# SuperScientificSoftwareLaboratory/TileSpMV

Measured on AMD Instinct MI355X. Metric: fp64 SpMV GFLOP/s (y = A*x, tiled format), higher is better.
Workload: dtype f64; 1 GPU; laplacian4096; rows=16777216, cols=16777216, nnz=83869696, partition=tile-row blocks, nnz-balanced, 1 rank(s), y_combine=none, tiles=5234176, x_panel_merge=0, x_slice_passes=0

## Files before the change

include/tilespmv.h:

```cpp
#ifndef TILESPMV_H_
#define TILESPMV_H_

#include <stddef.h>
#include <stdint.h>

#ifdef __cplusplus
extern "C" {
#endif

#ifndef MAT_VAL_TYPE
#define MAT_VAL_TYPE double
#endif
#ifndef MAT_PTR_TYPE
#define MAT_PTR_TYPE int
#endif

#define TILESPMV_BLOCK_SIZE 16
#define TILESPMV_COO_NNZ_TH 12
#define TILESPMV_PREFETCH_SMEM_TH 4

enum {
    TILESPMV_FMT_CSR = 0,
    TILESPMV_FMT_COO = 1,
    TILESPMV_FMT_ELL = 2,
// ... 240 lines not shown
    TILESPMV_INFO_WG_STRIPS = 16,
    TILESPMV_INFO_LIST_ENTRIES = 17,
    TILESPMV_INFO_DERIVED_UNITS = 18,
    TILESPMV_INFO_BRICK_ORDER = 19,
    TILESPMV_INFO_DESC_BYTES = 20,
    TILESPMV_INFO_NT_STREAM = 21,
    TILESPMV_INFO_UNIT_VALUE_BYTES = 22,
    TILESPMV_INFO_UNIT_LEAN = 23,
    TILESPMV_INFO_PLACEMENT_TRIES = 24,
    TILESPMV_INFO_RETIRED_25 = 25,
    TILESPMV_INFO_X_PANELS = 26,
    TILESPMV_INFO_X_PANEL_MERGE = 27,
    TILESPMV_INFO_SCATTERED_ENTRIES = 28,
    TILESPMV_INFO_X_SLICE_PASSES = 29,
    TILESPMV_INFO_CSR_FORM = 30,
    TILESPMV_INFO_TIMED_CHOICES_US = 31,
    TILESPMV_INFO_DEVICE_BUILD = 32,
    TILESPMV_INFO_TILE_CREATE_US = 33,
    TILESPMV_INFO_VALUE_MAP_BYTES = 34,
    TILESPMV_INFO_COUNT = 35
};
void tilespmv_plan_info(const tilespmv_plan *plan, long long *out );
int tilespmv_plan_strip_stride(const tilespmv_plan *plan);
long long tilespmv_plan_stream_digests(const tilespmv_plan *plan, unsigned long long *out , long long max_streams);

double tilespmv_plan_time(tilespmv_plan *plan, const MAT_VAL_TYPE *d_x, MAT_VAL_TYPE *d_y,
                          void *stream, int warmup, int reps);

double tilespmv_plan_time_reference_style(tilespmv_plan *plan, const MAT_VAL_TYPE *d_x, MAT_VAL_TYPE *d_y,
                                          void *stream, int reps);

void tilespmv_partition_tilerows(const Tile_matrix *matrix, int nparts, int *bounds);

int tilespmv_sizeof_value(void);

int tilespmv_reorder_rcm(int n, const MAT_PTR_TYPE *csrRowPtr, const int *csrColIdx, int *perm );
int tilespmv_csr_permute(int n, const MAT_PTR_TYPE *csrRowPtr, const int *csrColIdx, const MAT_VAL_TYPE *csrVal, const int *perm,
                         MAT_PTR_TYPE *outRowPtr , int *outColIdx, MAT_VAL_TYPE *outVal);
long long tilespmv_csr_bandwidth(int n, const MAT_PTR_TYPE *csrRowPtr, const int *csrColIdx);
int tilespmv_permute_vector(const MAT_VAL_TYPE *d_in, MAT_VAL_TYPE *d_out, const int *d_perm, long long n, int scatter, void *stream);

int tilespmv_csr_transpose(int rowA, int colA, const MAT_PTR_TYPE *csrRowPtr, const int *csrColIdx, const MAT_VAL_TYPE *csrVal ,
                           MAT_PTR_TYPE *rowPtrT , int *colIdxT, MAT_VAL_TYPE *valT , int *srcT );
int tilespmv_csr_transpose_device(int rowA, int colA, const MAT_PTR_TYPE *d_csrRowPtr, const int *d_csrColIdx, const MAT_VAL_TYPE *d_csrVal ,
                                  MAT_PTR_TYPE *d_rowPtrT, int *d_colIdxT, MAT_VAL_TYPE *d_valT , int *d_srcT , void *stream);

// ... 119 lines not shown
```

tilespmv_amd/_lib.py:

```python
import ctypes as C
import os
import subprocess

import numpy as np

from .tile_matrix import TileMatrixF32, TileMatrixF64

_ROOT = os.path.dirname(os.path.abspath(__file__))
_I = C.POINTER(C.c_int)
_U = C.POINTER(C.c_uint)
_CACHE = {}

INFO_NAMES = ["device_bytes", "stream_bytes", "nnz", "rows", "tiles", "coo_mode", "dense_mode", "kernel",
              "num_tasks", "num_split_rows", "fallback_nnz", "build_us", "upload_us", "entry_mode", "entry_ordered", "strip_cost",
              "wg_strips", "list_entries", "derived_units", "brick_order", "desc_bytes", "nt_stream", "unit_value_bytes", "unit_lean", "placement_tries", "retired_25", "x_panels", "x_panel_merge", "scattered_entries", "x_slice_passes", "csr_form", "timed_choices_us", "device_build", "tile_create_us",
              "value_map_bytes"]


BJ_INFO_NAMES = ["rows", "block_size", "blocks", "singular_blocks", "device_bytes", "dot_partials"]

FSAI_INFO_NAMES = ["rows", "nnz", "longest_row", "truncated_rows", "fallback_rows", "device_bytes", "dot_partials"]

KNOB_DEFAULT = -1
KNOB_NAMES = ["entry_mode", "entry_ordered", "strip_cost", "split_above", "split_cap", "xcd_remap", "xcd_chunk", "csr_split", "fix_inline",
# ... 94 lines not shown
    lib.tilespmv_plan_spmm.argtypes = [C.c_void_p, C.c_void_p, C.c_void_p, C.c_int, C.c_void_p]
    lib.tilespmv_plan_spmm.restype = C.c_int
    lib.tilespmv_plan_time_spmm.argtypes = [C.c_void_p, C.c_void_p, C.c_void_p, C.c_int, C.c_void_p, C.c_int, C.c_int]
    lib.tilespmv_plan_time_spmm.restype = C.c_double
    lib.tilespmv_plan_create.argtypes = [C.POINTER(C.c_void_p), TP, C.c_int, C.c_int, C.c_int, C.POINTER(PlanOptions)]
    lib.tilespmv_plan_create.restype = C.c_int
    lib.tilespmv_plan_options_init.argtypes = [C.POINTER(PlanOptions)]
    lib.tilespmv_plan_options_init.restype = None
    lib.tilespmv_plan_layout_digest.argtypes = [TP, C.c_int, C.c_int, C.c_int, C.POINTER(PlanOptions), C.POINTER(C.c_ulonglong), C.POINTER(C.c_longlong)]
    lib.tilespmv_plan_layout_digest.restype = C.c_int
    lib.tilespmv_plan_layout_stages.argtypes = [TP, C.c_int, C.c_int, C.c_int, C.POINTER(PlanOptions), C.POINTER(C.c_ulonglong), C.POINTER(C.c_longlong)]
    lib.tilespmv_plan_layout_stages.restype = C.c_int
    lib.tilespmv_plan_destroy.argtypes = [C.c_void_p]
    lib.tilespmv_plan_destroy.restype = None
    lib.tilespmv_plan_spmv.argtypes = [C.c_void_p, C.c_void_p, C.c_void_p, C.c_void_p]
    lib.tilespmv_plan_spmv.restype = C.c_int
    lib.tilespmv_plan_spmv_n.argtypes = [C.c_void_p, C.c_void_p, C.c_void_p, C.c_void_p, C.c_int]
    lib.tilespmv_plan_spmv_n.restype = C.c_int
    lib.tilespmv_plan_info.argtypes = [C.c_void_p, C.POINTER(C.c_longlong)]
    lib.tilespmv_plan_info.restype = None
    if hasattr(lib, "tilespmv_plan_strip_stride"):
        lib.tilespmv_plan_strip_stride.argtypes = [C.c_void_p]
        lib.tilespmv_plan_strip_stride.restype = C.c_int
    lib.tilespmv_plan_time.argtypes = [C.c_void_p, C.c_void_p, C.c_void_p, C.c_void_p, C.c_int, C.c_int]
    lib.tilespmv_plan_time.restype = C.c_double
    lib.tilespmv_plan_time_reference_style.argtypes = [C.c_void_p, C.c_void_p, C.c_void_p, C.c_void_p, C.c_int]
    lib.tilespmv_plan_time_reference_style.restype = C.c_double
    lib.tilespmv_plan_reserve_spmm.argtypes = [C.c_void_p, C.c_int]
    lib.tilespmv_plan_reserve_spmm.restype = C.c_int
    lib.tilespmv_partition_tilerows.argtypes = [TP, C.c_int, _I]
    lib.tilespmv_partition_tilerows.restype = None
    lib.tilespmv_matrix_save.argtypes = [TP, C.c_int, C.c_int, C.c_int, C.c_char_p]
    lib.tilespmv_matrix_save.restype = C.c_int
    lib.tilespmv_matrix_load.argtypes = [TP, _I, _I, _I, C.c_char_p]
    lib.tilespmv_matrix_load.restype = C.c_int
    lib.tilespmv_csr_save.argtypes = [C.c_char_p, C.c_int, C.c_int, C.c_int, C.c_int, _I, _I, VP, C.c_char_p]
    lib.tilespmv_csr_save.restype = C.c_int
    lib.tilespmv_csr_load.argtypes = [C.c_char_p, _I, _I, _I, _I, C.POINTER(_I), C.POINTER(_I), C.POINTER(VP), C.c_char_p]
    lib.tilespmv_csr_load.restype = C.c_int
    lib.mmio_allinone_cached.argtypes = [_I, _I, _I, _I, C.POINTER(_I), C.POINTER(_I), C.POINTER(VP), C.c_char_p, C.c_char_p, _I]
    lib.mmio_allinone_cached.restype = C.c_int
    lib.tilespmv_mtx_write.argtypes = [C.c_char_p, C.c_int, C.c_int, C.c_int, _I, _I, VP]
    lib.tilespmv_mtx_write.restype = C.c_int
    lib.tilespmv_reorder_rcm.argtypes = [C.c_int, _I, _I, _I]
    lib.tilespmv_reorder_rcm.restype = C.c_int
    lib.tilespmv_csr_permute.argtypes = [C.c_int, _I, _I, VP, _I, _I, _I, VP]
# ... 83 lines not shown
                    "tilespmv_device_count", "tilespmv_matrix_save", "tilespmv_matrix_load", "tilespmv_plan_spmv_n",
                    "call_tilespmv_hip_multi", "tilespmv_plan_spmm", "tilespmv_plan_time_spmm", "tilespmv_plan_options_init", "tilespmv_plan_layout_digest",
                    "tilespmv_csr_save", "tilespmv_csr_load", "mmio_allinone_cached", "tilespmv_mtx_write",
                    "tilespmv_plan_time_reference_style", "tilespmv_plan_reserve_spmm", "tilespmv_plan_options_layout", "tilespmv_plan_layout_stages",
                    "Tile_create_device", "tilespmv_plan_create_from_csr", "tilespmv_plan_stream_digests", "tilespmv_plan_create_from_device_csr",
                    "tilespmv_reorder_rcm", "tilespmv_csr_permute", "tilespmv_csr_bandwidth", "tilespmv_permute_vector",
                    "tilespmv_plan_update_values", "tilespmv_csr_transpose", "tilespmv_csr_transpose_device",
                    "tilespmv_cg_create", "tilespmv_cg_destroy", "tilespmv_cg_begin", "tilespmv_cg_iterate", "tilespmv_cg_state_read", "tilespmv_cg_solve",
                    "tilespmv_csr_diagonal_device",
                    "tilespmv_cg_multi_create", "tilespmv_cg_multi_destroy", "tilespmv_cg_multi_begin", "tilespmv_cg_multi_iterate", "tilespmv_cg_multi_state_read",
                    "tilespmv_cg_multi_solve",
                    "tilespmv_cgls_create", "tilespmv_cgls_destroy", "tilespmv_cgls_begin", "tilespmv_cgls_iterate", "tilespmv_cgls_state_read", "tilespmv_cgls_solve",
                    "tilespmv_csr_row_sqnorms_device",
                    "tilespmv_bicgstab_create", "tilespmv_bicgstab_destroy", "tilespmv_bicgstab_begin", "tilespmv_bicgstab_iterate", "tilespmv_bicgstab_state_read",
                    "tilespmv_bicgstab_solve",
                    "tilespmv_minres_create", "tilespmv_minres_destroy", "tilespmv_minres_begin", "tilespmv_minres_iterate", "tilespmv_minres_state_read", "tilespmv_minres_solve",
                    "tilespmv_csr_abs_diagonal_device",
                    "tilespmv_block_jacobi_create", "tilespmv_block_jacobi_destroy", "tilespmv_block_jacobi_update", "tilespmv_block_jacobi_apply", "tilespmv_block_jacobi_apply_dot",
                    "tilespmv_block_jacobi_info", "tilespmv_cg_create_block", "tilespmv_bicgstab_create_block",
                    "tilespmv_fsai_create", "tilespmv_fsai_destroy", "tilespmv_fsai_update", "tilespmv_fsai_apply", "tilespmv_fsai_apply_dot", "tilespmv_fsai_factor_csr",
                    "tilespmv_fsai_info", "tilespmv_cg_create_fsai",
                    "tilespmv_gmres_create", "tilespmv_gmres_create_block", "tilespmv_gmres_destroy", "tilespmv_gmres_begin", "tilespmv_gmres_iterate", "tilespmv_gmres_flush",
                    "tilespmv_gmres_state_read", "tilespmv_gmres_solve", "tilespmv_gmres_create_basis", "tilespmv_gmres_basis_bytes", "tilespmv_gmres_workspace_bytes",
                    "tilespmv_plan_strip_stride"]
```

tilespmv_amd/api.py:

```python
import ctypes as C

import numpy as np

from . import _lib
from .tile_matrix import to_dict

_I, _U = _lib._I, _lib._U

COO_AUTO, COO_IN_TILE, COO_FALLBACK = 0, 1, 2
DENSE_AUTO, DENSE_MFMA, DENSE_VALU = 0, 1, 2
KERNEL_AUTO, KERNEL_DIRECT, KERNEL_STREAM = 0, 1, 2
CREATE_HYB, CREATE_QUIET, CREATE_CDNA4, CREATE_VALUE_MAP = 1, 2, 4, 8
CREATE_TRANSPOSE = 16
ERR_NO_VALUE_MAP = -4


def _p(a, t):
    return a.ctypes.data_as(C.POINTER(t))


def _take(lib, ptr, n, dtype):
    if not ptr:
        return np.zeros(0, dtype=dtype)
    addr = C.cast(ptr, C.c_void_p).value
# ... 199 lines not shown

def csr_bandwidth(n, rowptr, colidx, dtype=np.float64):
    lib = _lib.load(dtype)
    rp, ci = np.ascontiguousarray(rowptr, dtype=np.int32), np.ascontiguousarray(colidx, dtype=np.int32)
    return int(lib.tilespmv_csr_bandwidth(n, _p(rp, C.c_int), _p(ci, C.c_int)))


def permute_vector(d_in, d_out, d_perm, n, scatter=False, stream=0, dtype=np.float64):
    rc = _lib.load(dtype).tilespmv_permute_vector(d_in, d_out, d_perm, n, 1 if scatter else 0, stream)
    if rc != 0:
        raise RuntimeError("tilespmv_permute_vector failed (hipError %d)" % rc)


def plan_layout_digest(tm, rowA, colA, nnzA, coo_mode=COO_AUTO, dense_mode=DENSE_AUTO, kernel=0, tilerow_begin=0, tilerow_end=0, **knobs):
    opts = _lib.PlanOptions(coo_mode, dense_mode, kernel, tilerow_begin, tilerow_end, False, **knobs)
    d = C.c_ulonglong(0)
    out = (C.c_longlong * len(_lib.INFO_NAMES))()
    rc = tm._lib.tilespmv_plan_layout_digest(C.byref(tm), rowA, colA, nnzA, C.byref(opts), C.byref(d), out)
    if rc != 0:
        raise RuntimeError("tilespmv_plan_layout_digest failed (%d)" % rc)
    return d.value, {k: int(out[i]) for i, k in enumerate(_lib.INFO_NAMES)}


STAGE_NAMES = ["count", "choose", "cut", "emit", "order", "encode", "entries", "finish"]


def plan_layout_stages(tm, rowA, colA, nnzA, coo_mode=COO_AUTO, dense_mode=DENSE_AUTO, kernel=0, tilerow_begin=0, tilerow_end=0, **knobs):
    opts = _lib.PlanOptions(coo_mode, dense_mode, kernel, tilerow_begin, tilerow_end, False, **knobs)
    st = (C.c_ulonglong * len(STAGE_NAMES))()
    out = (C.c_longlong * len(_lib.INFO_NAMES))()
    rc = tm._lib.tilespmv_plan_layout_stages(C.byref(tm), rowA, colA, nnzA, C.byref(opts), st, out)
    if rc != 0:
        raise RuntimeError("tilespmv_plan_layout_stages failed (%d)" % rc)
    return {k: int(st[i]) for i, k in enumerate(STAGE_NAMES)}, {k: int(out[i]) for i, k in enumerate(_lib.INFO_NAMES)}


class Plan:

    def __init__(self, tm, rowA, colA, nnzA, coo_mode=COO_AUTO, dense_mode=DENSE_AUTO, kernel=0, tilerow_begin=0, tilerow_end=0, autotune=False, **knobs):
        self.lib = tm._lib
        self.rowA, self.colA, self.nnzA = rowA, colA, nnzA
        self.shape = (rowA, colA)
        opts = _lib.PlanOptions(coo_mode, dense_mode, kernel, tilerow_begin, tilerow_end, autotune, **knobs)
        h = C.c_void_p()
        rc = self.lib.tilespmv_plan_create(C.byref(h), C.byref(tm), rowA, colA, nnzA, C.byref(opts))
        if rc != 0 or not h:
# ... 75 lines not shown
        if ms < 0:
            raise RuntimeError("tilespmv_plan_time failed")
        return ms

    def time_reference_style(self, d_x, d_y, stream=0, reps=100):
        ms = self.lib.tilespmv_plan_time_reference_style(self.h, C.c_void_p(d_x), C.c_void_p(d_y), C.c_void_p(stream), reps)
        if ms < 0:
            raise RuntimeError("tilespmv_plan_time_reference_style failed")
        return ms

    def reserve_spmm(self, nvec):
        rc = self.lib.tilespmv_plan_reserve_spmm(self.h, nvec)
        if rc != 0:
            raise RuntimeError("tilespmv_plan_reserve_spmm: HIP error %d" % rc)

    def info(self):
        out = (C.c_longlong * len(_lib.INFO_NAMES))()
        self.lib.tilespmv_plan_info(self.h, out)
        return {k: int(out[i]) for i, k in enumerate(_lib.INFO_NAMES)}

    def strip_stride(self):
        return int(self.lib.tilespmv_plan_strip_stride(self.h))

    def stream_digests(self):
        out = (C.c_ulonglong * (3 * 64))()
        n = self.lib.tilespmv_plan_stream_digests(self.h, out, 64)
        if n < 0 or n > 64:
            raise RuntimeError("tilespmv_plan_stream_digests failed (%d)" % n)
        return {int(out[3 * i]): (int(out[3 * i + 1]), int(out[3 * i + 2])) for i in range(n)}

    def close(self):
        if getattr(self, "h", None):
            self.lib.tilespmv_plan_destroy(self.h)
            self.h = None

    def __del__(self):
        try:
            self.close()
        except Exception:
            pass


CG_RUNNING, CG_CONVERGED, CG_MAXITER, CG_BREAKDOWN = 0, 1, 2, 3
CG_STATUS_NAMES = ["running", "converged", "maxiter", "breakdown"]
HIP_ERROR_INVALID_VALUE = 1

# ... 313 lines not shown
```

tilespmv_amd/csrc/hip_kernels.hip:

```cpp
#include <hip/hip_runtime.h>

#include "hip_plan.h"
#include "plan_tile_ops.h"
#include "hip_units_kernel.h"

namespace tilespmv {


typedef double v4d __attribute__((ext_vector_type(4)));
typedef float v4f __attribute__((ext_vector_type(4)));

constexpr int GROUPS_PER_BLOCK = 16;
#ifndef TILESPMV_STREAM_MIN_WAVES
#define TILESPMV_STREAM_MIN_WAVES 1
#endif

__device__ __forceinline__ int nibble_of(const unsigned char *__restrict__ base, int p)
{
    const unsigned b = base[p >> 1];
    return (p & 1) ? (int)(b & 15u) : (int)(b >> 4);
}

__device__ __forceinline__ void mfma_dense_tile(const val_t *__restrict__ tile, const val_t *xseg, int lane, val_t *out16)
{
// ... 1107 lines not shown
}

hipError_t launch_pair_values(const val_t *src, val_t *dst, const int4 *map, int ntasks, int narrow)
{
    if (ntasks > 0) hipLaunchKernelGGL(k_pair_values, dim3((unsigned)std::min(ntasks, 1 << 20)), dim3(256), 0, nullptr, src, dst, map, ntasks, narrow);
    return hipGetLastError();
}

hipError_t launch_tiles_stream(const DevPlan &P, const DevStream &S, const DevDense &DN, bool dense_mfma, int entry_mode, int wg_strips, int lds_pad_bytes, int xcd_remap, int xcd_chunk,
                               const val_t *x, val_t *y, hipStream_t st)
{
    if (S.ntasks > 0) {
        const int xc = xcd_remap == 2 ? xcd_chunk : 0;
#define TSPMV_KN(W, CD) hipLaunchKernelGGL((k_units<TILESPMV_UB, W, 16, CD, true, false, false, true>), dim3((unsigned)((S.ntasks + 15) / 16)), dim3(256), (size_t)lds_pad_bytes, st, S, P.rowA, P.colA, xc, P.partial, x, y)
#define TSPMV_K(W, B, CD, NTS, PL, WD) hipLaunchKernelGGL((k_units<TILESPMV_UB, W, B, CD, NTS, PL, WD>), dim3((unsigned)((S.ntasks + B - 1) / B)), dim3(16 * B), (size_t)lds_pad_bytes, st, S, P.rowA, P.colA, xc, P.partial, x, y)
#define TSPMV_NTS(W, B, CD, PL, WD) do { if (S.nt_stream) TSPMV_K(W, B, CD, true, PL, WD); else TSPMV_K(W, B, CD, false, PL, WD); } while (0)
#define TSPMV_FORM_(W, B, L) do { \
            if (S.pooled) { if (S.ucol) L(W, B, false, true, true); else if (S.pdict) L(W, B, true, true, false); else L(W, B, false, true, false); } \
            else if (S.cb_bits > 0) L(W, B, true, false, false); else L(W, B, false, false, false); } while (0)
#define TSPMV_PLAIN(W, B, CD, PL, WD) TSPMV_K(W, B, CD, false, PL, WD)
#define TSPMV_FORM(W, B) TSPMV_FORM_(W, B, TSPMV_NTS)
#define TSPMV_FORM_SMALL(W, B) TSPMV_FORM_(W, B, TSPMV_PLAIN)
        const bool small_grid = entry_mode != 2 && !S.nt_stream && (S.ntasks + 15) / 16 < SMALL_GRID_WORKGROUPS;
        if (const int lean = unit_lean_form(S, entry_mode, wg_strips)) {
            const hipError_t el = launch_units_lean(P, S, lean, entry_mode, wg_strips, lds_pad_bytes, xc, x, y, st);
            if (el != hipSuccess) return el;
        } else
#if !defined(TILESPMV_F32)
        if (S.uval_narrow == 2) {
            const hipError_t eh = launch_units_half(P, S, entry_mode, wg_strips, lds_pad_bytes, xc, x, y, st);
            if (eh != hipSuccess) return eh;
        } else if (S.uval_narrow) {
            if (S.pooled || !S.nt_stream || entry_mode == 1 || wg_strips != 16) return hipErrorInvalidValue;
            if (entry_mode == 2) { if (S.cb_bits > 0) TSPMV_KN(2, true); else TSPMV_KN(2, false); }
            else { if (S.cb_bits > 0) TSPMV_KN(0, true); else TSPMV_KN(0, false); }
        } else
#endif
        if (small_grid) { if (entry_mode == 1) TSPMV_FORM_SMALL(1, 8); else TSPMV_FORM_SMALL(0, 8); }
        else if (entry_mode == 1) TSPMV_FORM_SMALL(1, 16);
        else if (entry_mode == 2 && wg_strips == 32 && !S.pooled) {
            if (S.cb_bits > 0) TSPMV_NTS(2, 32, true, false, false); else TSPMV_NTS(2, 32, false, false, false);
        }
        else if (entry_mode == 2) TSPMV_FORM(2, 16);
        else TSPMV_FORM(0, 16);
#undef TSPMV_FORM_SMALL
#undef TSPMV_FORM
#undef TSPMV_PLAIN
// ... 21 lines not shown
```

tilespmv_amd/csrc/hip_plan.h:

```cpp
#pragma once
#include <cstdint>

#include "host_util.h"

namespace tilespmv {

constexpr unsigned DESC_FMT_MASK = 7u;
constexpr unsigned DESC_FMT_NOP = 7u;
constexpr unsigned DESC_EOR = 8u;
constexpr int DESC_P1_SHIFT = 4;
constexpr int DESC_P2_SHIFT = 12;

#if defined(TILESPMV_F32)
struct ERec { unsigned v, w; };
#else
struct ERec { unsigned lo, hi, w; };
#endif
constexpr int ECHUNK = 64;
constexpr int SMALL_GRID_WORKGROUPS = 128;
constexpr int FB_DEST_BITS = 11;

struct Task {
    int tile_begin, tile_end;
    long long val_off;
// ... 101 lines not shown
    int coo_heavy_min;
    int coo_ordered;
    int y_streaming;
    const int4 *wg_coo;
    const ERec *grec;
    const unsigned *gbase;
    int dest_bits;
    const uint4 *udict;
    int cb_bits;
    int nt_stream;
    int uval_narrow;
    const int *panel_off;
    int x_panels;
    int panel_merge;
    int n_groups;
    int slice_passes;
    int slice_ct;
    const UDesc *udesc_cb;
    const FixRow *ifix;
    unsigned *ifix_count;
    int unit_facts;
    int unit_lean;
    int strip_stride = 1;
};
constexpr int UNIT_FACT_NO_ROWUNIT = 1, UNIT_FACT_NO_DERIVED = 2;
inline int unit_lean_form(const DevStream &S, int entry_mode, int wg_strips)
{
    if (!S.unit_lean || S.ntasks <= 0 || S.pooled || !S.nt_stream || !(entry_mode == 0 || entry_mode == 2) || wg_strips != 16) return 0;
    if (!(S.unit_facts & UNIT_FACT_NO_ROWUNIT)) return 0;
    return (S.unit_facts & UNIT_FACT_NO_DERIVED) ? 2 : 1;
}

struct DenseRow { int row, tile_begin, tile_end, partial; };
__host__ __device__ constexpr int dense_slot(int r, int c)
{
    return sizeof(val_t) == 8 ? ((c & 3) >> 1) * 128 + ((c >> 2) * 16 + r) * 2 + (c & 1) : ((c >> 2) * 16 + r) * 4 + (c & 3);
}

struct DevDense {
    const int *cb;
    const val_t *val;
    const DenseRow *rows;
    int nrows;
};

inline void tile_stream_sizes(int fmt, int p1, int p2, int *nv, int *ni)
{
    switch (fmt) {
    case TILESPMV_FMT_CSR: *nv = p1; *ni = 16 + (p1 + 1) / 2; break;
    case TILESPMV_FMT_COO: *nv = p1; *ni = p1; break;
    case TILESPMV_FMT_ELL: *nv = 16 * p1; *ni = 8 * p1; break;
    case TILESPMV_FMT_HYB: *nv = 16 * p1 + p2; *ni = 8 * p1 + p2; break;
    case TILESPMV_FMT_DNS: *nv = 256; *ni = 0; break;
    case TILESPMV_FMT_DNSROW: *nv = 16 * p1; *ni = p1; break;
    case TILESPMV_FMT_DNSCOL: *nv = 16 * p1; *ni = p1; break;
    default: *nv = 0; *ni = 0; break;
    }
}

hipError_t launch_units_half(const DevPlan &P, const DevStream &S, int entry_mode, int wg_strips, int lds_pad_bytes, int xcd_chunk, const val_t *x, val_t *y, hipStream_t st);
hipError_t launch_units_lean(const DevPlan &P, const DevStream &S, int form, int entry_mode, int wg_strips, int lds_pad_bytes, int xcd_chunk, const val_t *x, val_t *y, hipStream_t st);

}
```

tilespmv_amd/csrc/hip_plan.hip:

```cpp
#include <type_traits>

#include "hip_plan_internal.h"
#include "hip_plan_device.h"
#include "tile_fields.h"

namespace tilespmv {
hipError_t launch_permute_vector(const val_t *in, val_t *out, const int *perm, long long n, int scatter, hipStream_t st);

hipError_t launch_tiles_direct(const DevPlan &P, bool dense_mfma, bool accumulate, bool fixup, const val_t *x, val_t *y, hipStream_t st);
hipError_t launch_tiles_stream(const DevPlan &P, const DevStream &S, const DevDense &DN, bool dense_mfma, int entry_mode, int wg_strips, int lds_pad_bytes, int xcd_remap, int xcd_chunk,
                               const val_t *x, val_t *y, hipStream_t st);
hipError_t launch_fallback(const DevPlan &P, const val_t *x, val_t *y, hipStream_t st);
hipError_t launch_tiles_stream_mv(const DevPlan &P, const DevStream &S, const DevDense &DN, int nvec, int xcd_chunk, bool entries_pass, int slab_rows, const val_t *X, val_t *Y,
                                  hipStream_t st);
hipError_t launch_rows_to_columns(const val_t *X, int nvec, long long n, long long ld, val_t *XT, hipStream_t st);
hipError_t launch_columns_to_rows(const val_t *YT, int nvec, long long row0, long long rows, long long ld, val_t *Y, hipStream_t st);

static Knobs resolve_knobs(const tilespmv_plan_options *opts)
{
    tilespmv_plan_options o;
    tilespmv_plan_options_init(&o);
    if (opts && opts->size >= sizeof(unsigned)) memcpy(&o, opts, std::min<size_t>(opts->size, sizeof(o)));
    o.size = (unsigned)sizeof(o);
    auto pick = [](int opt, const char *env, int dflt) { return opt != TILESPMV_KNOB_DEFAULT ? opt : env_int(env, dflt); };
// ... 16 lines not shown
    k.coo_cost = pick(o.coo_cost, "TILESPMV_COO_COST", 4);
    k.coo_heavy_min = std::max(0, pick(o.coo_heavy_min, "TILESPMV_COO_HEAVY_MIN", 32));
    k.coo_piece = pick(o.coo_piece, "TILESPMV_COO_PIECE", 0);
    k.strip_even = pick(o.strip_even, "TILESPMV_STRIP_EVEN", 4);
    k.wg_strips = pick(o.wg_strips, "TILESPMV_WG_STRIPS", -1);
    k.x_window = pick(o.x_window, "TILESPMV_X_WINDOW", -1);
    k.x_stride1 = pick(o.x_stride1, "TILESPMV_X_STRIDE1", 0);
    k.x_stride2 = pick(o.x_stride2, "TILESPMV_X_STRIDE2", 0);
    k.lds_pad = pick(o.lds_pad, "TILESPMV_LDS_PAD", -1);
    k.y_store = pick(o.y_store, "TILESPMV_Y_STORE", -1);
    k.mv_native = pick(o.mv_native, "TILESPMV_MV_NATIVE", -1);
    k.mv_xcd_chunk = pick(o.mv_xcd_chunk, "TILESPMV_MV_XCD_CHUNK", -1);
    k.desc_dict = pick(o.desc_dict, "TILESPMV_DESC_DICT", -1);
    k.nt_stream = pick(o.nt_stream, "TILESPMV_NT_STREAM", -1);
    k.placement_tries = pick(o.placement_tries, "TILESPMV_PLACEMENT_TRIES", -1);
    k.x_panel_kb = pick(o.x_panel_kb, "TILESPMV_X_PANEL_KB", -1);
    k.x_panel_merge = pick(o.x_panel_merge, "TILESPMV_X_PANEL_MERGE", -1);
    k.x_slice_passes = pick(o.x_slice_passes, "TILESPMV_X_SLICE_PASSES", -1);
    k.absorb = pick(o.absorb, "TILESPMV_ABSORB", -1); if (k.absorb < 0 || k.absorb > 2) k.absorb = 1;
    k.value_narrow = pick(o.value_narrow, "TILESPMV_VALUE_NARROW", -1);
    static const int unit_lean_env = env_int("TILESPMV_UNIT_LEAN", 1);
    k.unit_lean = (o.unit_lean != TILESPMV_KNOB_DEFAULT ? o.unit_lean : unit_lean_env) != 0 ? 1 : 0;
    k.strip_sweep = std::max(-1, std::min(1, env_int("TILESPMV_STRIP_SWEEP", -1)));
    k.deterministic = pick(o.deterministic, "TILESPMV_DETERMINISTIC", 0) > 0 ? 1 : 0;
    if (k.deterministic) {
        if (k.placement_tries < 0) k.placement_tries = 1;
        if (k.x_panel_merge < 0) k.x_panel_merge = 0;
        if (k.x_slice_passes < 0) k.x_slice_passes = 0;
        k.autotune = 0;
        k.entry_ordered = 1; k.x_slice_passes = 0;
    }
    k.xcd_from_caller = pinned(o.xcd_remap, "TILESPMV_XCD_REMAP") || pinned(o.xcd_chunk, "TILESPMV_XCD_CHUNK");
    k.entry_from_caller = pinned(o.entry_mode, "TILESPMV_WAVE_COO");
    k.strip_from_caller = o.strip_cost > 0 || env_int("TILESPMV_STRIP_COST", 0) > 0;
    k.autotune_log = getenv("TILESPMV_AUTOTUNE_LOG");
    k.verbose = getenv("TILESPMV_PLAN_VERBOSE") != nullptr;
    k.placement_force = env_int("TILESPMV_PLACEMENT_FORCE", 0) != 0;
    k.encode_check = env_int("TILESPMV_ENCODE_CHECK", 0) != 0;
    k.encode_on_host = env_int("TILESPMV_ENCODE_ON_HOST", 0) != 0;
    return k;
}

}

using namespace tilespmv;

// ... 619 lines not shown
        D.f_nblk = (int)f_blk.size();
        const int ordered_env = K.entry_ordered;
        D.f_ordered = ordered_env >= 0 ? ordered_env != 0 : f_blk.size() >= 2048;
    }
    if (rc) { tilespmv_plan_destroy(plan); return rc; }
    D.nfix = (int)fix.size();
    D.rowA = std::min<long long>(rowA, (long long)tr1 * 16); D.colA = colA;
    D.f_row0 = row0; D.f_rows = rows;
    plan->matrix_rows = rowA;

    long long *I = plan->info;
    I[TILESPMV_INFO_NNZ] = span(T->tile_nnz, DT ? DT->T.tile_nnz : nullptr, t_begin, t_end);
    I[TILESPMV_INFO_ROWS] = rows;
    I[TILESPMV_INFO_TILES] = t_end - t_begin;
    I[TILESPMV_INFO_COO_MODE] = coo_mode; I[TILESPMV_INFO_DENSE_MODE] = dense_mode; I[TILESPMV_INFO_KERNEL] = plan->kernel;
    I[TILESPMV_INFO_NUM_TASKS] = n_tasks; I[TILESPMV_INFO_NUM_SPLIT_ROWS] = (long long)fix.size();
    I[TILESPMV_INFO_FALLBACK_NNZ] = f_nnz;
    I[TILESPMV_INFO_UNIT_VALUE_BYTES] = plan->st.uval_narrow == 2 ? 2 : plan->st.uval_narrow ? 4 : sv;
    I[TILESPMV_INFO_UNIT_LEAN] = plan->kernel == TILESPMV_KERNEL_STREAM ? unit_lean_form(plan->st, plan->entry_mode, plan->wg_strips) : 0;
    if (plan->kernel != TILESPMV_KERNEL_STREAM) { I[TILESPMV_INFO_ENTRY_ORDERED] = 1; I[TILESPMV_INFO_STRIP_COST] = target; }
    I[TILESPMV_INFO_BUILD_US] = (long long)(now_us() - t_create0) - I[TILESPMV_INFO_UPLOAD_US];
    I[TILESPMV_INFO_STREAM_BYTES] = model_bytes + (long long)colA * sv + (long long)rows * sv +
                                    (f_nnz ? (long long)f_rec.size() * (long long)sizeof(ERec) + (long long)f_base.size() * 4 + 2LL * sv * rows + (long long)f_blk.size() * 16 : 0);
    if (!K.dry) {
        const int tries = K.placement_tries >= 0 ? K.placement_tries : (I[TILESPMV_INFO_DEVICE_BYTES] >= (1ll << 30) ? 8 : 1);
        const double t0p = now_us();
        retry_placement(plan, tries, K);
        I[TILESPMV_INFO_BUILD_US] += (long long)(now_us() - t0p);
        if (tries > 1 && !plan->arena_blocks.empty()) I[TILESPMV_INFO_TIMED_CHOICES_US] += (long long)(now_us() - t0p);
    }
    if (!K.dry && plan->panel_calibrate) {
        const double t0c = now_us();
        calibrate_panels(plan, colA, K.verbose);
        I[TILESPMV_INFO_BUILD_US] += (long long)(now_us() - t0c);
        I[TILESPMV_INFO_TIMED_CHOICES_US] += (long long)(now_us() - t0c);
    }
    if (plan->st.panel_merge > 0) {
        const int m = plan->st.panel_merge, passes = (plan->st.x_panels + m - 1) / m;
        I[TILESPMV_INFO_X_PANELS] = passes;
        I[TILESPMV_INFO_STREAM_BYTES] += 2LL * sv * plan->panel_rmw_rows / m + (passes - 1LL) * (n_tasks * 32 + (long long)plan->st.n_groups * 16);
    } else I[TILESPMV_INFO_X_PANELS] = 1;
    I[TILESPMV_INFO_X_PANEL_MERGE] = plan->st.panel_merge;
    I[TILESPMV_INFO_X_SLICE_PASSES] = plan->st.slice_passes;
    if (plan->st.slice_passes > 0) {
        I[TILESPMV_INFO_X_PANELS] = plan->st.slice_passes;
        I[TILESPMV_INFO_ENTRY_ORDERED] = 0;
// ... 199 lines not shown
{
    long long n = 0;
    std::vector<unsigned char> buf;
    for (size_t i = 0; i < plan->uploaded_slots.size(); i++) {
        const void *dev = *plan->uploaded_slots[i];
        const size_t bytes = plan->uploaded_bytes[i];
        unsigned long long h = 1469598103934665603ull;
        if (bytes && dev) {
            buf.resize(bytes);
            if (hipMemcpy(buf.data(), dev, bytes, hipMemcpyDeviceToHost) != hipSuccess) { (void)hipGetLastError(); return -3; }
            for (size_t q = 0; q < bytes; q++) { h ^= buf[q]; h *= 1099511628211ull; }
        }
        if (n < max_streams) { out[3 * n] = (unsigned long long)((const char *)plan->uploaded_slots[i] - (const char *)plan); out[3 * n + 1] = bytes; out[3 * n + 2] = h; }
        n++;
    }
    return n;
}

int tilespmv_plan_strip_stride(const tilespmv_plan *plan)
{
    return plan->kernel == TILESPMV_KERNEL_STREAM ? std::max(1, plan->st.strip_stride) : 1;
}

void tilespmv_plan_info(const tilespmv_plan *plan, long long *out)
{
    memcpy(out, plan->info, sizeof(plan->info));
}

double tilespmv_plan_time(tilespmv_plan *plan, const MAT_VAL_TYPE *d_x, MAT_VAL_TYPE *d_y, void *stream, int warmup, int reps)
{
    hipStream_t st = (hipStream_t)stream;
    hipEvent_t a = nullptr, b = nullptr;
    if (hipEventCreate(&a) != hipSuccess) return -1.0;
    if (hipEventCreate(&b) != hipSuccess) { (void)hipEventDestroy(a); return -1.0; }
    bool ok = true;
    for (int i = 0; ok && i < warmup; i++) ok = tilespmv_plan_spmv(plan, d_x, d_y, stream) == 0;
    if (ok) ok = hipEventRecord(a, st) == hipSuccess;
    for (int i = 0; ok && i < reps; i++) ok = tilespmv_plan_spmv(plan, d_x, d_y, stream) == 0;
    if (ok) ok = hipEventRecord(b, st) == hipSuccess && hipEventSynchronize(b) == hipSuccess;
    float ms = 0.f;
    if (ok) ok = hipEventElapsedTime(&ms, a, b) == hipSuccess;
    (void)hipEventDestroy(a); (void)hipEventDestroy(b);
    if (!ok) return -1.0;
    return reps > 0 ? (double)ms / reps : 0.0;
}

// ... 66 lines not shown
```

tilespmv_amd/csrc/hip_plan_internal.h:

```cpp
#pragma once
#include <hip/hip_runtime.h>
#include <sys/time.h>

#include <climits>
#include <cmath>
#include <string>
#include <unordered_map>
#include <unordered_set>

#include "hip_plan.h"
#include "plan_tile_ops.h"

#define HIP_TRY(expr)                                                                                   \
    do {                                                                                                \
        hipError_t e_ = (expr);                                                                         \
        if (e_ != hipSuccess) {                                                                         \
            fprintf(stderr, "tilespmv: HIP error %d (%s) at %s:%d: %s\n", (int)e_, hipGetErrorString(e_), \
                    __FILE__, __LINE__, #expr);                                                         \
            return (int)e_;                                                                             \
        }                                                                                               \
    } while (0)

namespace tilespmv {

// ... 14 lines not shown
    int coo_mode, dense_mode, kernel, tilerow_begin, tilerow_end, autotune;
    int entry_mode;
    int entry_ordered;
    int strip_cost;
    int split_above, split_cap, xcd_remap, xcd_chunk, csr_split, fix_inline, coo_cost, coo_heavy_min;
    int coo_piece;
    int strip_even;
    int wg_strips;
    int x_window;
    int x_stride1, x_stride2;
    int lds_pad;
    int y_store;
    int mv_native;
    int mv_xcd_chunk;
    int nt_stream;
    int x_panel_kb;
    int x_panel_merge;
    int x_slice_passes;
    int placement_tries;
    int deterministic;
    int absorb;
    int unit_lean;
    int strip_sweep;
    int value_narrow;
    bool value_map;
    int desc_dict;
    bool xcd_from_caller, entry_from_caller, strip_from_caller;
    bool dry;
    const char *autotune_log;
    bool verbose;
    bool placement_force;
    bool encode_check;
    bool encode_on_host;
};

}

using namespace tilespmv;

static inline int slice_trip_records(long long list_records, int groups, int passes)
{
    const double avg = (double)list_records / std::max(1.0, 8.0 * passes * (double)std::max(1, groups));
    return avg * 1.1 <= 1024 ? 4 : avg * 1.1 <= 1536 ? 6 : 8;
}

struct tilespmv_plan {
// ... 226 lines not shown
```

Baseline: 1658 GFLOP/s.

## Add deep-pipelined unit kernel with double-buffered gathers and value loads

Adds a new stream-unit SpMV kernel that keeps two batches of four units in flight. Descriptor chunks are refilled inside LDS while x gathers and value loads for the next batch are issued before the current batch is multiplied, to hide memory latency. It is enabled by default on large streaming plans that have no list entries, fixups or fallback blocks, and can be forced on or off with an environment variable. In exchange it raises register pressure, and the launch bounds ask for fewer waves per SIMD, so occupancy may drop.

```diff
diff --git a/include/tilespmv.h b/include/tilespmv.h
--- a/include/tilespmv.h
+++ b/include/tilespmv.h
@@ -286,6 +286,8 @@
 };
 void tilespmv_plan_info(const tilespmv_plan *plan, long long *out );
 int tilespmv_plan_strip_stride(const tilespmv_plan *plan);
+int tilespmv_plan_unit_deep(const tilespmv_plan *plan);
+int tilespmv_plan_layout_unit_deep(const Tile_matrix *matrix, int rowA, int colA, MAT_PTR_TYPE nnzA, const tilespmv_plan_options *opts);
 long long tilespmv_plan_stream_digests(const tilespmv_plan *plan, unsigned long long *out , long long max_streams);
 
 double tilespmv_plan_time(tilespmv_plan *plan, const MAT_VAL_TYPE *d_x, MAT_VAL_TYPE *d_y,
diff --git a/tilespmv_amd/_lib.py b/tilespmv_amd/_lib.py
--- a/tilespmv_amd/_lib.py
+++ b/tilespmv_amd/_lib.py
@@ -140,6 +140,11 @@
     if hasattr(lib, "tilespmv_plan_strip_stride"):
         lib.tilespmv_plan_strip_stride.argtypes = [C.c_void_p]
         lib.tilespmv_plan_strip_stride.restype = C.c_int
+    if hasattr(lib, "tilespmv_plan_unit_deep"):
+        lib.tilespmv_plan_unit_deep.argtypes = [C.c_void_p]
+        lib.tilespmv_plan_unit_deep.restype = C.c_int
+        lib.tilespmv_plan_layout_unit_deep.argtypes = [TP, C.c_int, C.c_int, C.c_int, C.POINTER(PlanOptions)]
+        lib.tilespmv_plan_layout_unit_deep.restype = C.c_int
     lib.tilespmv_plan_time.argtypes = [C.c_void_p, C.c_void_p, C.c_void_p, C.c_void_p, C.c_int, C.c_int]
     lib.tilespmv_plan_time.restype = C.c_double
     lib.tilespmv_plan_time_reference_style.argtypes = [C.c_void_p, C.c_void_p, C.c_void_p, C.c_void_p, C.c_int]
@@ -269,4 +274,4 @@
                     "tilespmv_fsai_info", "tilespmv_cg_create_fsai",
                     "tilespmv_gmres_create", "tilespmv_gmres_create_block", "tilespmv_gmres_destroy", "tilespmv_gmres_begin", "tilespmv_gmres_iterate", "tilespmv_gmres_flush",
                     "tilespmv_gmres_state_read", "tilespmv_gmres_solve", "tilespmv_gmres_create_basis", "tilespmv_gmres_basis_bytes", "tilespmv_gmres_workspace_bytes",
-                    "tilespmv_plan_strip_stride"]
+                    "tilespmv_plan_strip_stride", "tilespmv_plan_unit_deep", "tilespmv_plan_layout_unit_deep"]
diff --git a/tilespmv_amd/api.py b/tilespmv_amd/api.py
--- a/tilespmv_amd/api.py
+++ b/tilespmv_amd/api.py
@@ -245,6 +245,14 @@
     return d.value, {k: int(out[i]) for i, k in enumerate(_lib.INFO_NAMES)}
 
 
+def plan_layout_unit_deep(tm, rowA, colA, nnzA, coo_mode=COO_AUTO, dense_mode=DENSE_AUTO, kernel=0, tilerow_begin=0, tilerow_end=0, **knobs):
+    opts = _lib.PlanOptions(coo_mode, dense_mode, kernel, tilerow_begin, tilerow_end, False, **knobs)
+    rc = tm._lib.tilespmv_plan_layout_unit_deep(C.byref(tm), rowA, colA, nnzA, C.byref(opts))
+    if rc < 0:
+        raise RuntimeError("tilespmv_plan_layout_unit_deep failed (%d)" % rc)
+    return int(rc)
+
+
 STAGE_NAMES = ["count", "choose", "cut", "emit", "order", "encode", "entries", "finish"]
 
 
@@ -366,6 +374,9 @@
     def strip_stride(self):
         return int(self.lib.tilespmv_plan_strip_stride(self.h))
 
+    def unit_deep(self):
+        return int(self.lib.tilespmv_plan_unit_deep(self.h))
+
     def stream_digests(self):
         out = (C.c_ulonglong * (3 * 64))()
         n = self.lib.tilespmv_plan_stream_digests(self.h, out, 64)
diff --git a/tilespmv_amd/csrc/hip_kernels.hip b/tilespmv_amd/csrc/hip_kernels.hip
--- a/tilespmv_amd/csrc/hip_kernels.hip
+++ b/tilespmv_amd/csrc/hip_kernels.hip
@@ -1153,7 +1153,10 @@
 #define TSPMV_FORM(W, B) TSPMV_FORM_(W, B, TSPMV_NTS)
 #define TSPMV_FORM_SMALL(W, B) TSPMV_FORM_(W, B, TSPMV_PLAIN)
         const bool small_grid = entry_mode != 2 && !S.nt_stream && (S.ntasks + 15) / 16 < SMALL_GRID_WORKGROUPS;
-        if (const int lean = unit_lean_form(S, entry_mode, wg_strips)) {
+        if (const int deep = unit_deep_form(S, entry_mode, wg_strips)) {
+            const hipError_t ed = launch_units_deep(P, S, deep, entry_mode, wg_strips, lds_pad_bytes, xc, x, y, st);
+            if (ed != hipSuccess) return ed;
+        } else if (const int lean = unit_lean_form(S, entry_mode, wg_strips)) {
             const hipError_t el = launch_units_lean(P, S, lean, entry_mode, wg_strips, lds_pad_bytes, xc, x, y, st);
             if (el != hipSuccess) return el;
         } else
diff --git a/tilespmv_amd/csrc/hip_kernels_deep.hip b/tilespmv_amd/csrc/hip_kernels_deep.hip
--- /dev/null
+++ b/tilespmv_amd/csrc/hip_kernels_deep.hip
@@ -0,0 +1,177 @@
+#include <hip/hip_runtime.h>
+
+#include "hip_plan.h"
+#include "hip_plan_internal.h"
+#include "hip_units_kernel.h"
+
+namespace tilespmv {
+
+constexpr int deep_min_waves(int vf) { return sizeof(val_t) == 4 ? 8 : vf == 2 ? 7 : vf == 1 ? 6 : 5; }
+
+template <int UB, int DEPTH, bool CD, int VF, bool DERIVED>
+__global__ __launch_bounds__(256, deep_min_waves(VF)) void k_units_deep(DevStream S, int rowA, int colA, int xcd_chunk, const val_t *__restrict__ x, val_t *__restrict__ y)
+{
+    static_assert(UB == 4 && DEPTH == 2, "the one form that was kept (DESIGN.md S8 item 15): two batches of 4 units in flight, whose buffers take turns inside a chunk of 4 batches");
+    static_assert(VF >= 0 && VF <= (sizeof(val_t) == 8 ? 2 : 0), "a value form of this build");
+    constexpr int G = VF != 0 ? UNIT_GROUP_NARROW : UNIT_GROUP;
+    constexpr int NG = UB / G;
+    static_assert(DCHUNK % UB == 0 && UB % G == 0, "a batch never straddles a descriptor chunk and is whole value groups");
+    __shared__ lacc_t s_yall[16 * STRIP_MAX_ROWS * 16];
+    lacc_t (*s_y)[STRIP_MAX_ROWS][16] = reinterpret_cast<lacc_t (*)[STRIP_MAX_ROWS][16]>(&s_yall[0]);
+    __shared__ uint4 s_d[16][DCHUNK];
+    const int tid = threadIdx.x, r = tid & 15, g = tid >> 4;
+    unsigned bid = blockIdx.x;
+    if (xcd_chunk > 0) {
+        const unsigned C = (unsigned)xcd_chunk, W = 8u * C, win = bid / W, off = bid % W, k = off & 7u;
+        if ((win + 1) * W <= gridDim.x) bid = win * W + k * C + (off >> 3);
+    }
+    const long long task_id = (long long)bid * 16 + g;
+    if (task_id >= S.ntasks) return;
+    const int4 t0 = reinterpret_cast<const int4 *>(S.task)[task_id * 2], t1 = reinterpret_cast<const int4 *>(S.task)[task_id * 2 + 1];
+    const int unit_begin = t0.x, unit_end = t0.y, row0 = t1.x, nrows = t1.w;
+    const unsigned nounit = (unsigned)t1.z;
+    typedef std::conditional_t<VF == 2, _Float16, std::conditional_t<VF == 1, float, val_t>> sval_t;
+    typedef sval_t grp_t __attribute__((ext_vector_type(G)));
+    const grp_t *__restrict__ ugrp = reinterpret_cast<const grp_t *>(S.uval) + r;
+    const grp_t *__restrict__ vhot = reinterpret_cast<const grp_t *>(S.uval);
+    const int xlast32 = colA - 1;
+    const unsigned *__restrict__ udw = reinterpret_cast<const unsigned *>(S.udesc);
+    const uint2 *sd = reinterpret_cast<const uint2 *>(&s_d[g][0]) + (r >> 3);
+
+    val_t acc = 0;
+    auto retire = [&](val_t prod, unsigned flags) {
+#pragma clang fp contract(off)
+        acc += prod;
+        if (flags & UNIT_EOR) {
+            const int kr = (int)((flags >> UNIT_ROW_SHIFT) & 7u);
+            if constexpr (sizeof(val_t) == sizeof(lacc_t)) s_y[g][kr][r] = acc;
+            else reinterpret_cast<val_t *>(&s_y[g][kr][0])[r] = acc;
+            acc = 0;
+        }
+    };
+
+    if (unit_begin < unit_end) {
+        const int last = unit_end - 1;
+        uint4 dcur = make_uint4(0u, 0u, 0u, 0u), dnext = dcur;
+        unsigned wnn = 0;
+        if constexpr (CD) { dcur.x = udw[min(unit_begin + r, last)]; dnext.x = udw[min(unit_begin + DCHUNK + r, last)]; }
+        else { dcur = load_udesc_raw(S.udesc, min(unit_begin + r, last)); dnext = load_udesc_raw(S.udesc, min(unit_begin + DCHUNK + r, last)); }
+        grp_t vs[2][NG];
+        auto load_values = [&](const int u0, const grp_t *p, grp_t (&out)[NG]) {
+#pragma unroll
+            for (int q = 0; q < NG; q++) out[q] = stream_load<true>((u0 + q * G < unit_end) ? p + q * 16 : vhot);
+        };
+        load_values(unit_begin, ugrp + (long long)unit_begin * (16 / G), vs[0]);
+        if constexpr (CD) {
+            const uint4 p0 = udict_of(S, dcur.x), p1 = udict_of(S, dnext.x);
+            wnn = udw[min(unit_begin + 2 * DCHUNK + r, last)];
+            dnext.y = p1.x; dnext.z = p1.z; dnext.w = p1.y;
+            s_d[g][r] = udesc_expand(S, dcur.x, p0);
+        } else s_d[g][r] = udesc_park_form(dcur);
+        wave_lds_fence();
+        constexpr int NB = DCHUNK / UB;
+        int cload = unit_begin + 2 * DCHUNK + r + 1;
+        unsigned w0[DEPTH][UB];
+        val_t xv[DEPTH][UB];
+        auto gather = [&](const int j0, unsigned (&w)[UB], val_t (&xg)[UB]) {
+#pragma unroll
+            for (int k = 0; k < UB; k++) {
+                const uint2 dk = sd[2 * (j0 + k)];
+                w[k] = dk.x;
+                xg[k] = x[x_index32(unit_x_base32(dk.x), (dk.y >> (28 - 4 * (r & 7))) & 15u, xlast32)];
+            }
+        };
+        auto refill = [&]() {
+            wave_lds_fence();
+            if constexpr (CD) s_d[g][r] = udesc_expand(S, dnext.x, make_uint4(dnext.y, dnext.w, dnext.z, 0u));
+            else s_d[g][r] = udesc_park_form(dnext);
+            wave_lds_fence();
+            if constexpr (CD) {
+                const uint4 p = udict_of(S, wnn);
+                dnext = make_uint4(wnn, p.x, p.z, p.y);
+                wnn = udw[min(cload + DCHUNK, unit_end) - 1];
+            } else dnext = load_udesc_raw(S.udesc, min(cload, unit_end) - 1);
+            cload += DCHUNK;
+        };
+        val_t xprev = 0;
+        int u = unit_begin;
+        auto multiply = [&](const unsigned (&w)[UB], const val_t (&xg)[UB], const grp_t (&vg)[NG], auto tail) {
+#pragma clang fp contract(off)
+#pragma unroll
+            for (int k = 0; k < UB; k++) {
+                val_t xu = xg[k];
+                if constexpr (DERIVED) { xu = unit_x_use(xg[k], xprev, w[k], r); xprev = xu; }
+                if (!decltype(tail)::value || u + k < unit_end) retire((val_t)vg[k / G][k % G] * xu, w[k] >> 24);
+            }
+        };
+        const grp_t *vnext = ugrp + (long long)(unit_begin + UB) * (16 / G);
+        auto step = [&](auto j_) {
+            constexpr int j = decltype(j_)::value, jg = (j + 1) % NB;
+            gather(jg * UB, w0[jg % DEPTH], xv[jg % DEPTH]);
+            load_values(u + UB, vnext, vs[(j + 1) % 2]);
+            vnext += UB * (16 / G);
+            if constexpr (jg == NB - 1) refill();
+            __builtin_amdgcn_sched_barrier(0);
+            multiply(w0[j % DEPTH], xv[j % DEPTH], vs[j % 2], std::false_type());
+            u += UB;
+        };
+        const int ulast = unit_begin + (unit_end - 1 - unit_begin) / UB * UB;
+        gather(0, w0[0], xv[0]);
+        while (u + (NB - 1) * UB < ulast) {
+            step(std::integral_constant<int, 0>());
+            step(std::integral_constant<int, 1>());
+            step(std::integral_constant<int, 2>());
+            step(std::integral_constant<int, 3>());
+        }
+        auto rest = [&](auto self, auto j_) -> void {
+            constexpr int j = decltype(j_)::value;
+            if constexpr (j + 1 < NB) {
+                if (u < ulast) { step(j_); self(self, std::integral_constant<int, j + 1>()); return; }
+            }
+            multiply(w0[j % DEPTH], xv[j % DEPTH], vs[j % 2], std::true_type());
+        };
+        rest(rest, std::integral_constant<int, 0>());
+    }
+    for (unsigned m = nounit; m; m &= m - 1) {
+        const int kr = __ffs((int)m) - 1;
+        if constexpr (sizeof(val_t) == sizeof(lacc_t)) s_y[g][kr][r] = 0;
+        else reinterpret_cast<val_t *>(&s_y[g][kr][0])[r] = 0;
+    }
+    wave_lds_fence();
+    constexpr int VEC = 16 / (int)sizeof(val_t);
+    constexpr int ROWV = 128 / (int)sizeof(val_t);
+    const val_t *res = reinterpret_cast<const val_t *>(&s_y[g][0][0]);
+    const int ystride = S.strip_stride;
+    for (int i = r * VEC; i < 16 * nrows; i += 16 * VEC) {
+        const long long yi = ((long long)row0 + (long long)(i >> 4) * ystride) * 16 + (i & 15);
+        const val_t *rf = res + (i >> 4) * ROWV + (i & 15);
+        if (yi + VEC <= rowA) {
+            if (NT_Y && S.y_streaming) __builtin_nontemporal_store(*reinterpret_cast<const v4u_t *>(rf), reinterpret_cast<v4u_t *>(y + yi));
+            else *reinterpret_cast<uint4 *>(y + yi) = *reinterpret_cast<const uint4 *>(rf);
+        } else {
+#pragma unroll
+            for (int q = 0; q < VEC; q++) if (yi + q < rowA) y[yi + q] = rf[q];
+        }
+    }
+}
+
+hipError_t launch_units_deep(const DevPlan &P, const DevStream &S, int depth, int entry_mode, int wg_strips, int lds_pad_bytes, int xcd_chunk, const val_t *x, val_t *y, hipStream_t st)
+{
+    if (depth != unit_deep_form(S, entry_mode, wg_strips) || depth < 1) return hipErrorInvalidValue;
+    const bool derived = unit_lean_form(S, entry_mode, wg_strips) == 1;
+#define TSPMV_KD(CD, VF, DV) hipLaunchKernelGGL((k_units_deep<UNIT_DEEP_UB, UNIT_DEEP_DEPTH, CD, VF, DV>), dim3((unsigned)((S.ntasks + 15) / 16)), dim3(256), (size_t)lds_pad_bytes, st, S, P.rowA, P.colA, xcd_chunk, x, y)
+#define TSPMV_KD_DV(CD, VF) do { if (derived) TSPMV_KD(CD, VF, true); else TSPMV_KD(CD, VF, false); } while (0)
+#define TSPMV_KD_CD(VF) do { if (S.cb_bits > 0) TSPMV_KD_DV(true, VF); else TSPMV_KD_DV(false, VF); } while (0)
+#if !defined(TILESPMV_F32)
+    if (S.uval_narrow == 2) TSPMV_KD_CD(2);
+    else if (S.uval_narrow == 1) TSPMV_KD_CD(1);
+    else
+#endif
+    TSPMV_KD_CD(0);
+#undef TSPMV_KD_CD
+#undef TSPMV_KD_DV
+#undef TSPMV_KD
+    return hipGetLastError();
+}
+
+}
diff --git a/tilespmv_amd/csrc/hip_plan.h b/tilespmv_amd/csrc/hip_plan.h
--- a/tilespmv_amd/csrc/hip_plan.h
+++ b/tilespmv_amd/csrc/hip_plan.h
@@ -147,6 +147,7 @@
     int unit_facts;
     int unit_lean;
     int strip_stride = 1;
+    int unit_deep = 0;
 };
 constexpr int UNIT_FACT_NO_ROWUNIT = 1, UNIT_FACT_NO_DERIVED = 2;
 inline int unit_lean_form(const DevStream &S, int entry_mode, int wg_strips)
@@ -154,6 +155,12 @@
     if (!S.unit_lean || S.ntasks <= 0 || S.pooled || !S.nt_stream || !(entry_mode == 0 || entry_mode == 2) || wg_strips != 16) return 0;
     if (!(S.unit_facts & UNIT_FACT_NO_ROWUNIT)) return 0;
     return (S.unit_facts & UNIT_FACT_NO_DERIVED) ? 2 : 1;
+}
+constexpr int UNIT_DEEP_UB = 4, UNIT_DEEP_DEPTH = 2;
+inline int unit_deep_form(const DevStream &S, int entry_mode, int wg_strips)
+{
+    if (!S.unit_deep || entry_mode != 0 || wg_strips != 16 || unit_lean_form(S, entry_mode, wg_strips) <= 0) return 0;
+    return UNIT_DEEP_DEPTH;
 }
 
 struct DenseRow { int row, tile_begin, tile_end, partial; };
@@ -185,5 +192,6 @@
 
 hipError_t launch_units_half(const DevPlan &P, const DevStream &S, int entry_mode, int wg_strips, int lds_pad_bytes, int xcd_chunk, const val_t *x, val_t *y, hipStream_t st);
 hipError_t launch_units_lean(const DevPlan &P, const DevStream &S, int form, int entry_mode, int wg_strips, int lds_pad_bytes, int xcd_chunk, const val_t *x, val_t *y, hipStream_t st);
+hipError_t launch_units_deep(const DevPlan &P, const DevStream &S, int depth, int entry_mode, int wg_strips, int lds_pad_bytes, int xcd_chunk, const val_t *x, val_t *y, hipStream_t st);
 
 }
diff --git a/tilespmv_amd/csrc/hip_plan.hip b/tilespmv_amd/csrc/hip_plan.hip
--- a/tilespmv_amd/csrc/hip_plan.hip
+++ b/tilespmv_amd/csrc/hip_plan.hip
@@ -62,6 +62,7 @@
     static const int unit_lean_env = env_int("TILESPMV_UNIT_LEAN", 1);
     k.unit_lean = (o.unit_lean != TILESPMV_KNOB_DEFAULT ? o.unit_lean : unit_lean_env) != 0 ? 1 : 0;
     k.strip_sweep = std::max(-1, std::min(1, env_int("TILESPMV_STRIP_SWEEP", -1)));
+    k.unit_deep = std::max(-1, std::min(1, env_int("TILESPMV_UNIT_DEEP", -1)));
     k.deterministic = pick(o.deterministic, "TILESPMV_DETERMINISTIC", 0) > 0 ? 1 : 0;
     if (k.deterministic) {
         if (k.placement_tries < 0) k.placement_tries = 1;
@@ -727,6 +728,8 @@
     I[TILESPMV_INFO_BUILD_US] = (long long)(now_us() - t_create0) - I[TILESPMV_INFO_UPLOAD_US];
     I[TILESPMV_INFO_STREAM_BYTES] = model_bytes + (long long)colA * sv + (long long)rows * sv +
                                     (f_nnz ? (long long)f_rec.size() * (long long)sizeof(ERec) + (long long)f_base.size() * 4 + 2LL * sv * rows + (long long)f_blk.size() * 16 : 0);
+    plan->st.unit_deep = (plan->kernel == TILESPMV_KERNEL_STREAM && K.unit_deep != 0 && I[TILESPMV_INFO_LIST_ENTRIES] == 0 && fix.empty() && f_blk.empty() &&
+                          (K.unit_deep > 0 || I[TILESPMV_INFO_STREAM_BYTES] > NT_STREAM_MIN_BYTES)) ? 1 : 0;
     if (!K.dry) {
         const int tries = K.placement_tries >= 0 ? K.placement_tries : (I[TILESPMV_INFO_DEVICE_BYTES] >= (1ll << 30) ? 8 : 1);
         const double t0p = now_us();
@@ -972,6 +975,23 @@
     return plan->kernel == TILESPMV_KERNEL_STREAM ? std::max(1, plan->st.strip_stride) : 1;
 }
 
+int tilespmv_plan_unit_deep(const tilespmv_plan *plan)
+{
+    return plan->kernel == TILESPMV_KERNEL_STREAM ? unit_deep_form(plan->st, plan->entry_mode, plan->wg_strips) : 0;
+}
+
+int tilespmv_plan_layout_unit_deep(const Tile_matrix *T, int rowA, int colA, MAT_PTR_TYPE nnzA, const tilespmv_plan_options *opts)
+{
+    Knobs K = resolve_knobs(opts);
+    K.dry = true; K.autotune = 0;
+    tilespmv_plan *p = nullptr;
+    const int rc = plan_create_one(&p, T, rowA, colA, nnzA, K);
+    if (rc != 0 || !p) return rc ? (rc < 0 ? rc : -rc) : -4;
+    const int deep = tilespmv_plan_unit_deep(p);
+    tilespmv_plan_destroy(p);
+    return deep;
+}
+
 void tilespmv_plan_info(const tilespmv_plan *plan, long long *out)
 {
     memcpy(out, plan->info, sizeof(plan->info));
diff --git a/tilespmv_amd/csrc/hip_plan_internal.h b/tilespmv_amd/csrc/hip_plan_internal.h
--- a/tilespmv_amd/csrc/hip_plan_internal.h
+++ b/tilespmv_amd/csrc/hip_plan_internal.h
@@ -60,6 +60,7 @@
     int absorb;
     int unit_lean;
     int strip_sweep;
+    int unit_deep;
     int value_narrow;
     bool value_map;
     int desc_dict;
```

Measured after the change: 1747 GFLOP/s, median of 6. 1.05x the previous value.
